# imazen/image-webp

Hardware: AMD Instinct MI355X
Metric: 1920x1080 lossy encodes/s (Q75, method 4) (higher is better)
Workload: dtype int32; 1 GPU; encode_frame_lossy 1920x1080 RGBA Q75 m4; device_batch=1024, distinct_frames=4, mbs_per_frame=8160, parallelism=frames sharded over 1 GPU(s), steps_pipelined=True, pipeline_lanes=2

## Files before the change

image-webp_amd/csrc/zw_dev.h:

```cpp
#pragma once
#include <hip/hip_runtime.h>
#include <stdint.h>
#include "zw_common.h"

#define ZW_TABLE(T, N, D, ...) __constant__ T d_##N D = {__VA_ARGS__};
#include "zw_tables.inc"
#undef ZW_TABLE

__constant__ uint8_t d_I4_IDX[10][16] = {
    {255, 255, 255, 255, 255, 255, 255, 255, 255, 255, 255, 255, 255, 255, 255, 255},
    {254, 254, 254, 254, 254, 254, 254, 254, 254, 254, 254, 254, 254, 254, 254, 254},
    {17, 18, 19, 20, 17, 18, 19, 20, 17, 18, 19, 20, 17, 18, 19, 20},
    {15, 15, 15, 15, 14, 14, 14, 14, 13, 13, 13, 13, 37, 37, 37, 37},
    {18, 19, 20, 21, 19, 20, 21, 22, 20, 21, 22, 23, 21, 22, 23, 36},
    {16, 17, 18, 19, 15, 16, 17, 18, 14, 15, 16, 17, 13, 14, 15, 16},
    {28, 29, 30, 31, 16, 17, 18, 19, 15, 28, 29, 30, 14, 16, 17, 18},
    {29, 30, 31, 32, 18, 19, 20, 21, 30, 31, 32, 22, 19, 20, 21, 23},
    {27, 16, 17, 18, 26, 15, 27, 16, 25, 14, 26, 15, 24, 13, 25, 14},
    {26, 14, 25, 13, 25, 13, 24, 37, 24, 37, 0, 0, 0, 0, 0, 0},
};

#define DI __device__ __forceinline__

DI int kZZ(int n) { return (int)((0xfeb7adc963258410ull >> (4 * n)) & 15); }
DI int kBand(int n)
{
    return n >= 16 ? 0 : (int)((0x7666666665463210ull >> (4 * n)) & 15);
}
DI int kWTrellis(int j)
{
    const unsigned long long lo = 0x0a11181b0b131b1eull, hi = 0x06080a0b080c1113ull;
    return (int)(((j < 8 ? lo : hi) >> (8 * (j & 7))) & 255);
}
DI int kWY(int j)
{
    const unsigned long long lo = 0x07111c2009142026ull, hi = 0x02040709040a1114ull;
    return (int)(((j < 8 ? lo : hi) >> (8 * (j & 7))) & 255);
}

DI int band_of(int n)
{
    return n >= 16 ? 0 : (int)((0x7666666665463210ull >> (4 * n)) & 15);
}
DI int zz_of(int n) { return (int)((0xfeb7adc963258410ull >> (4 * n)) & 15); }
DI int izz_of(int k) { return (int)((0xfea9db83c7426510ull >> (4 * k)) & 15); }

DI int clamp255(int v) { return v < 0 ? 0 : (v > 255 ? 255 : v); }
DI int iabs(int v) { return v < 0 ? -v : v; }

__device__ __forceinline__ int pk_y(uint32_t p)
{
    return (16839 * (int)(p & 255u) + 33059 * (int)((p >> 8) & 255u) + 6420 * (int)((p >> 16) & 255u) + (1 << 15) +
            (16 << 16)) >> 16;
}
__device__ __forceinline__ int pk_u(uint32_t p)
{
    return -9719 * (int)(p & 255u) - 19081 * (int)((p >> 8) & 255u) + 28800 * (int)((p >> 16) & 255u);
}
__device__ __forceinline__ int pk_v(uint32_t p)
{
    return 28800 * (int)(p & 255u) - 24116 * (int)((p >> 8) & 255u) - 4684 * (int)((p >> 16) & 255u);
}
__device__ __forceinline__ uint32_t udot2(uint32_t a, uint32_t b, uint32_t c)
{
    uint32_t d;
    asm("v_dot2_u32_u16 %0, %1, %2, %3" : "=v"(d) : "v"(a), "v"(b), "v"(c));
    return d;
}
__device__ __forceinline__ int sdot2(uint32_t a, uint32_t b, int c)
{
    int d;
    asm("v_dot2_i32_i16 %0, %1, %2, %3" : "=v"(d) : "v"(a), "v"(b), "v"(c));
    return d;
}
__device__ __forceinline__ uint32_t pk_y2(uint32_t p)
{
    const uint32_t rg = __builtin_amdgcn_perm(0u, p, 0x0c010c00u);
    return udot2(rg, 0x812341c7u , ((p >> 16) & 255u) * 6420u + (1u << 15) + (16u << 16)) >> 16;
}
__device__ __forceinline__ uint32_t pk_y4(uint32_t p0, uint32_t p1, uint32_t p2, uint32_t p3)
{
    auto y = [](uint32_t p) {
        const uint32_t hi = __builtin_amdgcn_udot4(p, 0x00198141u, 0u, false);
        const uint32_t lo = __builtin_amdgcn_udot4(p, 0x001423c7u, (1u << 15) + (16u << 16), false);
        return (hi << 8) + lo;
    };
    const uint32_t lo = __builtin_amdgcn_perm(y(p1), y(p0), 0x0c0c0602u);
    const uint32_t hi = __builtin_amdgcn_perm(y(p3), y(p2), 0x06020c0cu);
    return lo | hi;
}
__device__ __forceinline__ void pk_uv4(uint32_t a, uint32_t b, uint32_t c, uint32_t d, uint32_t& u, uint32_t& v)
{
    const uint32_t sel = 0x0c020c00u;
    const uint32_t rb = __builtin_amdgcn_perm(0u, a, sel) + __builtin_amdgcn_perm(0u, b, sel) +
                        __builtin_amdgcn_perm(0u, c, sel) + __builtin_amdgcn_perm(0u, d, sel);
    const int g = (int)(((a >> 8) & 255u) + ((b >> 8) & 255u) + ((c >> 8) & 255u) + ((d >> 8) & 255u));
    const int su = sdot2(rb, 0x7080da09u , g * -19081 + (512 << 16));
    const int sv = sdot2(rb, 0xedb47080u , g * -24116 + (512 << 16));
    u = (uint32_t)((su + (1 << 17)) >> 18);
    v = (uint32_t)((sv + (1 << 17)) >> 18);
}

DI void wsync()
// ... 117 lines not shown
        b[r * 4] = w16(a + d) >> 3;
        b[r * 4 + 1] = w16(bb + c) >> 3;
        b[r * 4 + 2] = w16(bb - c) >> 3;
        b[r * 4 + 3] = w16(a - d) >> 3;
    }
}

DI void wht16(int* b)
{
#pragma unroll
    for (int i = 0; i < 4; i++) {
        int a = b[i * 4] + b[i * 4 + 3], bb = b[i * 4 + 1] + b[i * 4 + 2];
        int c = b[i * 4 + 1] - b[i * 4 + 2], d = b[i * 4] - b[i * 4 + 3];
        b[i * 4] = a + bb;
        b[i * 4 + 1] = c + d;
        b[i * 4 + 2] = a - bb;
        b[i * 4 + 3] = d - c;
    }
#pragma unroll
    for (int i = 0; i < 4; i++) {
        int a1 = b[i] + b[i + 12], b1 = b[i + 4] + b[i + 8];
        int c1 = b[i + 4] - b[i + 8], d1 = b[i] - b[i + 12];
        int a2 = a1 + b1, b2 = c1 + d1, c2 = a1 - b1, d2 = d1 - c1;
        b[i] = (a2 + (a2 > 0 ? 1 : 0)) / 2;
        b[i + 4] = (b2 + (b2 > 0 ? 1 : 0)) / 2;
        b[i + 8] = (c2 + (c2 > 0 ? 1 : 0)) / 2;
        b[i + 12] = (d2 + (d2 > 0 ? 1 : 0)) / 2;
    }
}

DI void iwht16(int* b)
{
#pragma unroll
    for (int i = 0; i < 4; i++) {
        int a1 = b[i] + b[12 + i], b1 = b[4 + i] + b[8 + i];
        int c1 = b[4 + i] - b[8 + i], d1 = b[i] - b[12 + i];
        b[i] = a1 + b1;
        b[4 + i] = c1 + d1;
        b[8 + i] = a1 - b1;
        b[12 + i] = d1 - c1;
    }
#pragma unroll
    for (int r = 0; r < 4; r++) {
        int a1 = b[4 * r] + b[4 * r + 3], b1 = b[4 * r + 1] + b[4 * r + 2];
        int c1 = b[4 * r + 1] - b[4 * r + 2], d1 = b[4 * r] - b[4 * r + 3];
        b[4 * r] = (a1 + b1 + 3) >> 3;
        b[4 * r + 1] = (c1 + d1 + 3) >> 3;
        b[4 * r + 2] = (a1 - b1 + 3) >> 3;
        b[4 * r + 3] = (d1 - c1 + 3) >> 3;
    }
}

DI int ttransform(const int* in)
{
    int tmp[16];
#pragma unroll
    for (int i = 0; i < 4; i++) {
        const int* r = in + i * 4;
        int a0 = r[0] + r[2], a1 = r[1] + r[3], a2 = r[1] - r[3], a3 = r[0] - r[2];
        tmp[i * 4] = a0 + a1;
        tmp[i * 4 + 1] = a3 + a2;
        tmp[i * 4 + 2] = a3 - a2;
        tmp[i * 4 + 3] = a0 - a1;
    }
    int sum = 0;
#pragma unroll
    for (int i = 0; i < 4; i++) {
        int a0 = tmp[i] + tmp[8 + i], a1 = tmp[4 + i] + tmp[12 + i];
        int a2 = tmp[4 + i] - tmp[12 + i], a3 = tmp[i] - tmp[8 + i];
        sum += kWY(i) * iabs(a0 + a1) + kWY(4 + i) * iabs(a3 + a2) +
               kWY(8 + i) * iabs(a3 - a2) + kWY(12 + i) * iabs(a0 - a1);
    }
    return sum;
}

struct LdsTables {
    uint16_t lc[4][8][3][68];
    uint16_t eob[4][8][3];
    uint16_t init[4][8][3];
    uint8_t probs[4][8][3][11];
    uint16_t lfc[2048];
    uint16_t ent[256];
    uint16_t fci4[10][10][10];
    uint8_t i4idx[10][16];
    uint8_t i4qa[10][16];
    uint8_t zz[16];
    uint8_t bands[17];
    uint8_t izz[16];
    uint8_t pad[15];
    uint16_t beob[4][8][3];
    uint16_t binit[4][8][3];
};

DI void load_static_tables(LdsTables* T, int tid, int nt, const uint8_t* probs )
{
    for (int i = tid; i < 96; i += nt) {
        const int p0 = probs[i * 11];
        (&T->beob[0][0][0])[i] = d_VP8_ENTROPY_COST[p0];
        (&T->binit[0][0][0])[i] = d_VP8_ENTROPY_COST[255 - p0];
    }
    for (int i = tid; i < 2048; i += nt) T->lfc[i] = d_VP8_LEVEL_FIXED_COSTS[i];
    for (int i = tid; i < 256; i += nt) T->ent[i] = d_VP8_ENTROPY_COST[i];
    for (int i = tid; i < 1000; i += nt) (&T->fci4[0][0][0])[i] = (&d_VP8_FIXED_COSTS_I4[0][0][0])[i];
    for (int i = tid; i < 160; i += nt) {
        const int idx = (&d_I4_IDX[0][0])[i], p = i & 15;
        (&T->i4idx[0][0])[i] = (uint8_t)idx;
        (&T->i4qa[0][0])[i] = (uint8_t)(4 * (idx == 254 ? 3 - (p >> 2) : (idx == 255 ? 38 : idx)));
    }
    for (int i = tid; i < 16; i += nt) T->zz[i] = d_ZIGZAG[i];
    for (int i = tid; i < 17; i += nt) T->bands[i] = d_VP8_ENC_BANDS[i];
    for (int i = tid; i < 16; i += nt) T->izz[d_ZIGZAG[i]] = (uint8_t)i;
}

DI uint32_t bitcost(const LdsTables* T, int bit, int p) { return bit ? T->ent[255 - p] : T->ent[p]; }

template <int FIRST>
DI uint32_t rcost(const int* c, int ctx0, int ctype, const LdsTables* T)
{
    int last = -1;
#pragma unroll
    for (int n = 0; n < 16; n++)
        if (c[n] != 0) last = n;
    const int p0 = T->probs[ctype][kBand(FIRST)][ctx0][0];
    if (last < 0) return bitcost(T, 0, p0);
    uint32_t cost = ctx0 == 0 ? bitcost(T, 1, p0) : 0;
    int ctx = ctx0;
#pragma unroll
    for (int n = FIRST; n < 16; n++) {
        if (n <= last) {
            int v = iabs(c[n]);
            cost += T->lfc[v < 2047 ? v : 2047] + T->lc[ctype][kBand(n)][ctx][v < 67 ? v : 67];
            ctx = v < 2 ? v : 2;
        }
    }
    if (last < 15) cost += bitcost(T, 0, T->probs[ctype][band_of(last + 1)][ctx][0]);
    return cost;
}

#define DPP(v, ctrl) __builtin_amdgcn_mov_dpp((v), (ctrl), 0xf, 0xf, false)
DI int qb0(int v) { return DPP(v, 0x00); }
DI int qb1(int v) { return DPP(v, 0x55); }
DI int qb2(int v) { return DPP(v, 0xAA); }
DI int qb3(int v) { return DPP(v, 0xFF); }
DI int ror4(int v) { return DPP(v, 0x124); }
DI int ror8(int v) { return DPP(v, 0x128); }
DI int ror12(int v) { return DPP(v, 0x12C); }
DI int shr1(int v) { return __builtin_amdgcn_update_dpp(0, (v), 0x111, 0xf, 0xf, false); }
DI int red16(int v)
{
    v += DPP(v, 0xB1);
    v += DPP(v, 0x4E);
    v += DPP(v, 0x141);
    v += DPP(v, 0x140);
    return v;
}
DI int gget(int v, int k) { return __shfl(v, k, 16); }

DI int csel(bool c, int a, int b) { return b + ((a - b) & -(int)c); }

DI int sel4(int i, int a, int b, int c, int d)
{
    const int m0 = -(int)(i == 0), m1 = -(int)(i == 1), m2 = -(int)(i == 2), m3 = -(int)(i == 3);
    return (a & m0) | (b & m1) | (c & m2) | (d & m3);
}

DI void gcol(int t, int i, int& t0, int& t1, int& t2, int& t3)
{
    const int m1 = ror4(t), p2 = ror8(t), p1 = ror12(t);
    t0 = sel4(i, t, m1, p2, p1);
    t1 = sel4(i, p1, t, m1, p2);
    t2 = sel4(i, p2, p1, t, m1);
    t3 = sel4(i, m1, p2, p1, t);
}

DI int qrev(int v) { return DPP(v, 0x1B); }
DI int qnext(int v) { return DPP(v, 0x39); }
DI int qprev(int v) { return DPP(v, 0x93); }
DI int qxor2(int v) { return DPP(v, 0x4E); }
DI int rrev(int v) { return DPP(DPP(v, 0x140), 0x1B); }

DI int fdct_g(int v, int k)
{
    const int i = k >> 2, j = k & 3;
    {
        const int r = qrev(v);
        const int s = v + r, d = v - r;
        const int X = qnext(s), Y = qprev(d);
        const int ev = csel(j == 0, s + X, X - s) * 8;
        const int od = (m24(Y, 8 * 5352) + m24(d, csel(j == 1, 8 * 2217, -8 * 2217)) + csel(j == 1, 14500, 7500)) >> 12;
        v = csel((j & 1) == 0, ev, od);
// ... 532 lines not shown
```

image-webp_amd/csrc/zw_enc_i4pair.h:

```cpp
#pragma once
#include <stdint.h>

#ifndef ZW_HD
#ifdef __HIPCC__
#define ZW_HD __host__ __device__
#else
#define ZW_HD
#endif
#endif

#ifndef ZW_I4P_INV
#define ZW_I4P_INV 1
#endif
#ifndef ZW_I4P_LANES
#define ZW_I4P_LANES 1
#endif

#define ZW_I4P_KMAX 4

ZW_HD inline int i4p_inv_dest(int lane, int rank)
{
    return (lane & ~15) + (rank < ZW_I4P_KMAX ? 4 * rank : 1);
}
ZW_HD inline int i4p_mode_src(int lane) { return lane & ~3; }
ZW_HD inline bool i4p_eligible(int lane, int K) { return ((lane >> 2) & 3) < K; }
ZW_HD inline int i4p_mode(int lane, int K, int received) { return i4p_eligible(lane, K) ? received : 0; }

struct I4PWin {
    uint32_t pk;
    uint32_t sm;
};
ZW_HD inline I4PWin i4p_win(uint32_t rate, uint32_t mcost, bool nz, uint32_t sse, int mode)
{
    I4PWin w;
    w.pk = (rate & 0xffffu) | (mcost << 16) | ((uint32_t)nz << 31);
    w.sm = sse | ((uint32_t)mode << 24);
    return w;
}

struct I4PState {
    uint64_t running;
    uint32_t total_mc;
    uint32_t nzt;
    uint32_t lm;
};

ZW_HD inline void i4p_state_init(I4PState& s, uint32_t l_mode)
{
    s.running = 211ull * l_mode;
    s.total_mc = 0;
    s.nzt = 0;
    s.lm = 0;
}

ZW_HD inline void i4p_state_update(I4PState& s, int bx, int by, I4PWin w, uint32_t l_mode)
{
    const uint32_t mode = w.sm >> 24, sse = w.sm & 0xffffffu;
    s.nzt |= (w.pk >> 31) << (by * 4 + bx);
    s.nzt = (s.nzt & ~(0xf0000u << (4 * bx))) | (mode << (16 + 4 * bx));
    s.lm = (s.lm & ~(0xfu << (4 * by))) | (mode << (4 * by));
    s.total_mc += (w.pk >> 16) & 0x7fffu;
    s.running += (uint64_t)sse * 256ull + (uint64_t)(w.pk & 0xffffu) * l_mode;
}

ZW_HD inline int i4p_tctx(const I4PState& s, int bx, int by)
{
    return by == 0 ? 0 : (int)((s.nzt >> (16 + 4 * bx)) & 15u);
}
ZW_HD inline int i4p_lctx(const I4PState& s, int bx, int by)
{
    return bx == 0 ? 0 : (int)((s.lm >> (4 * by)) & 15u);
}
ZW_HD inline int i4p_nzctx(const I4PState& s, int bx, int by)
{
    const int i = by * 4 + bx;
    return (by == 0 ? 0 : (int)((s.nzt >> ((i - 4) & 15)) & 1u)) + (bx == 0 ? 0 : (int)((s.nzt >> ((i - 1) & 15)) & 1u));
}

ZW_HD inline bool i4p_exit(const I4PState& s, uint64_t i16_score)
{
    return s.running >= i16_score || s.total_mc > 256u * 16u * 16u / 4u;
}
```

image-webp_amd/csrc/zw_enc_kernels.hip:

```cpp
#include "zw_dev.h"

#include <type_traits>

#include "zw_enc_rows.h"
#include "zw_enc_pairfinal.h"
#include "zw_enc_i4pair.h"

#define ZW_PH_N 28

#ifdef ZW_NW
#define ZW_NW1 ZW_NW
#define ZW_NW2 ZW_NW
#endif
#ifndef ZW_NW1
#define ZW_NW1 12
#endif
#ifndef ZW_NW2
#define ZW_NW2 12
#endif
#define NW_MAX (ZW_NW1 > ZW_NW2 ? ZW_NW1 : ZW_NW2)
#ifndef ZW_DYN_PRIO
#define ZW_DYN_PRIO 1
#endif
#ifndef ZW_DYN_PRIO1
// ... 228 lines not shown
#ifdef ZW_PHASE_PROF
__device__ unsigned long long zw_phase_cycles_dev[2][ZW_PH_N];
__device__ unsigned long long zw_wave_cycles_dev[2][16][ZW_PH_N];
#define PH_START() long long ph_t_ = clock64()
#define PH_RESET() (ph_t_ = clock64())
#define PH_MARK(k) PH_MARK_L(k, lane, PASS)
#define PH_MARK_L(k, ln, ps)                                                        \
    do {                                                                            \
        const long long n_ = clock64();                                             \
        if ((ln) == 0) C.W->ph[k] += (unsigned long long)(n_ - ph_t_);               \
        ph_t_ = n_;                                                                 \
    } while (0)
extern "C" int zw_wave_cycles(unsigned long long* out, int reset)
{
    if (hipMemcpyFromSymbol(out, HIP_SYMBOL(zw_wave_cycles_dev), sizeof(zw_wave_cycles_dev)) != hipSuccess) return -1;
    if (reset) {
        static unsigned long long z[2][16][ZW_PH_N];
        if (hipMemcpyToSymbol(HIP_SYMBOL(zw_wave_cycles_dev), z, sizeof z) != hipSuccess) return -1;
    }
    return 0;
}
extern "C" int zw_phase_cycles(unsigned long long* out, int reset)
{
    if (hipMemcpyFromSymbol(out, HIP_SYMBOL(zw_phase_cycles_dev), sizeof(zw_phase_cycles_dev)) != hipSuccess) return -1;
    if (reset) {
        static unsigned long long z[2][ZW_PH_N];
        if (hipMemcpyToSymbol(HIP_SYMBOL(zw_phase_cycles_dev), z, sizeof z) != hipSuccess) return -1;
    }
    return 0;
}
#define PH_COUNT(k) \
    do {                \
        if (C.lane == 0) C.W->ph[k] += 1; \
    } while (0)
#else
#define PH_COUNT(k) (void)0
#define PH_START() (void)0
#define PH_RESET() (void)0
#define PH_MARK(k) (void)0
#define PH_MARK_L(k, ln, ps) (void)0
#endif

template <int NB>
__device__ __forceinline__ void i4_values_n(const Ctx& C, const int* x0, const int* y0)
{
    WaveLds* W = C.W;
    const uint8_t* ws = C.M->ws;
    const int l = C.lane;
    const int t = (int)(l >= 13) + (int)(l >= 24) + (int)(l >= 36) + (int)(l >= 37);
    const int k = min(l - 13 * (int)(l >= 13) - 11 * (int)(l >= 24), 12);
    const int t3 = (int)(t == 3), t4 = (int)(t >= 4), t12 = (int)(t == 1 || t == 2);
    const int ka = k + t3 * (11 - k) + t4 * (1 - k);
    const int kb = k + t12 + t3 * (12 - k) - t4 * k;
    const int kc = min(k + 2 * (int)(t == 1), 12);
    const int wb = 2 * (int)(t == 1) + (int)(t == 2) + 3 * (t3 + t4);
    const int wc = (int)(t == 1);
    const int sh = (int)(t != 0) + (int)(t != 0 && t != 2);
    const int oa = csel(ka < 4, -ka * ZW_BPS, ka - 4 - 4 * ZW_BPS);
    const int ob = csel(kb < 4, -kb * ZW_BPS, kb - 4 - 4 * ZW_BPS);
    const int oc = csel(kc < 4, -kc * ZW_BPS, kc - 4 - 4 * ZW_BPS);
    const bool dcl = l < 4 || (l >= 5 && l < 9);
    int v[NB], ea[NB];
#pragma unroll
    for (int h = 0; h < NB; h++) {
        const int rowL = (y0[h] + 3) * ZW_BPS + x0[h] - 1;
        ea[h] = ws[rowL + oa];
        const int eb = ws[rowL + ob], ec = ws[rowL + oc];
        v[h] = (ea[h] + wb * eb + wc * ec + ((1 << sh) >> 1)) >> sh;
    }
#pragma unroll
    for (int h = 0; h < NB; h++) {
        const int dsum = red16(dcl ? ea[h] : 0);
        if (l < 38) W->V[h][l] = v[h];
        if (l == 0) W->V[h][38] = (dsum + 4) >> 3;
    }
    wsync();
}
__device__ __forceinline__ void i4_values(const Ctx& C, int x0, int y0) { i4_values_n<1>(C, &x0, &y0); }

__device__ __forceinline__ int bperm(int v, int src_lane) { return __builtin_amdgcn_ds_bpermute(src_lane << 2, v); }

__device__ __forceinline__ int i4_src_index(const LdsTables* T, int mode, int p)
{
    const int idx = T->i4idx[mode][p];
    const bool tm = idx == 254;
    return csel(tm, 256 + 3 - (p >> 2), csel(idx == 255, 38, idx));
}
__device__ __forceinline__ int i4_pred_at(const int* V, int sidx, int vbc)
{
    const int va = V[sidx & 255];
    return csel(sidx >= 256, clamp255(va + vbc), va);
}

__device__ __forceinline__ unsigned long long rdscore(uint32_t sse, uint32_t rate, uint32_t lambda)
{
    return (unsigned long long)sse * 256ull + (unsigned long long)(uint16_t)rate * lambda;
}

struct I4State {
    unsigned long long running;
    uint32_t total_mc;
    unsigned long long mpack;
    uint32_t tnz, lnz;
    uint32_t nzm;
};

DI uint32_t min16u(uint32_t v)
{
    v = min(v, (uint32_t)DPP((int)v, 0x128));
    v = min(v, (uint32_t)DPP((int)v, 0x124));
    v = min(v, (uint32_t)DPP((int)v, 0x122));
    v = min(v, (uint32_t)DPP((int)v, 0x121));
    return v;
}

__device__ __forceinline__ int hx_partner(int v)
{
    const auto r = __builtin_amdgcn_permlane32_swap(v, v, false, false);
    return (__lane_id() < 32) ? (int)r[1] : (int)r[0];
}
__device__ __forceinline__ int hx_sum(int v)
{
    const auto r = __builtin_amdgcn_permlane32_swap(v, v, false, false);
    return (int)r[0] + (int)r[1];
}
DI int lo16(uint32_t v) { return (int)(int16_t)(v & 0xffffu); }
DI int hi16(uint32_t v) { return (int)(int16_t)(v >> 16); }

DI void uv_rows_pk(const uint8_t* w, const uint8_t* sblk, int bx, int by, int h, int m, int dc, uint32_t s01[2],
                   uint32_t s32[2], uint32_t p01[2], uint32_t p32[2])
{
    const int cm = -(int)(m & 1), rm = -(int)(m >= 2);
    const int P = w[0];
    const int ro = csel(m == 0, dc, csel(m == 3, -P, 0));
    const uint8_t* tp = w + 1 + bx * 4;
    const uint32_t c01 = pack_lo(tp[0] & cm, tp[1] & cm), c32 = pack_lo(tp[3] & cm, tp[2] & cm);
#pragma unroll
    for (int r = 0; r < 2; r++) {
        const int y = 2 * h + r;
        const int rv = (w[(by * 4 + y + 1) * ZW_BPS] & rm) + ro;
        const uint32_t rvv = pack_lo(rv, rv);
        p01[r] = clamp_pk(add_pk(c01, rvv));
        p32[r] = clamp_pk(add_pk(c32, rvv));
        const uint32_t sw = *(const uint32_t*)(sblk + y * 8);
        s01[r] = __builtin_amdgcn_perm(0u, sw, 0x0c010c00u);
        s32[r] = __builtin_amdgcn_perm(0u, sw, 0x0c020c03u);
    }
}

DI void fdct_pair(const uint32_t s01[2], const uint32_t s32[2], const uint32_t p01[2], const uint32_t p32[2], int h,
                  int cf[2][4])
{
    const zs2 k8p = {8, 8}, k8m = {8, -8}, k1a = {10704, 4434}, k1b = {4434, -10704};
    const uint32_t kA0 = h ? as_zu(k8m) : as_zu(k8p), kA1 = h ? as_zu(k8p) : as_zu(k8m);
    const uint32_t kD0 = h ? as_zu(k1b) : as_zu(k1a), kD1 = h ? as_zu(k1a) : as_zu(k1b);
    const int rD0 = h ? 1875 : 3625, rD1 = h ? 3625 : 1875;
    int own0[2], own1[2], oth0[2], oth1[2];
#pragma unroll
    for (int r = 0; r < 2; r++) {
        const uint32_t R01 = sub_pk(s01[r], p01[r]), R32 = sub_pk(s32[r], p32[r]);
        const uint32_t A = add_pk(R01, R32), D = sub_pk(R01, R32);
        own0[r] = dot2v(A, kA0, 0);
        oth0[r] = dot2v(A, kA1, 0);
        own1[r] = dot2v(D, kD0, rD0) >> 10;
        oth1[r] = dot2v(D, kD1, rD1) >> 10;
    }
    const uint32_t g0 = (uint32_t)hx_partner((int)pack_lo(oth0[0], oth0[1]));
    const uint32_t g1 = (uint32_t)hx_partner((int)pack_lo(oth1[0], oth1[1]));
    const zs2 k1p = {1, 1}, k1m = {1, -1}, k2a = {5352, 2217}, k2b = {2217, -5352};
// ... 523 lines not shown
    const uint32_t score = (uint32_t)sse * 256u + (rate & 0xffffu) * S.l_i4;
    const bool elig = m < 10 && rank < K;
    const uint32_t sk = elig ? score : 0xffffffffu;
    const uint32_t smin = min16u(sk);
    const uint32_t rk = sk == smin ? (uint32_t)rank : 0xffffffffu;
    const uint32_t rmin = min16u(rk);
    const unsigned long long win = __ballot(rk == rmin && sk == smin);
    PH_MARK_L(12, l, 0);
    int bmode[NB];
#pragma unroll
    for (int h = 0; h < NB; h++) {
        bmode[h] = __builtin_ctz((uint32_t)(win >> (16 * h)) & 0xffffu);
        const int wl = 16 * h + bmode[h];
        const uint32_t bsse = (uint32_t)__builtin_amdgcn_readlane(sse, wl);
        const uint32_t brate = (uint32_t)__builtin_amdgcn_readlane((int)rate, wl);
        const int bnz = __builtin_amdgcn_readlane((int)(last >= 0), wl);
        const int i = sby[h] * 4 + sbx[h];
        st.tnz = (st.tnz & ~(1u << sbx[h])) | ((uint32_t)bnz << sbx[h]);
        st.lnz = (st.lnz & ~(1u << sby[h])) | ((uint32_t)bnz << sby[h]);
        st.nzm |= (uint32_t)bnz << i;
        st.total_mc += (uint32_t)__builtin_amdgcn_readlane(mcost, wl);
        st.running += rdscore(bsse, brate, S.l_mode);
        st.mpack |= (unsigned long long)bmode[h] << (4 * i);
        if (l == h) C.M->modes[i] = (uint8_t)bmode[h];
    }
    const int bms = csel(slot, bmode[sl], bmode[0]);
    if (m == bms && (NB == 2 || slot == 0)) {
        const int xo = csel(slot, x0[sl], x0[0]), yo = csel(slot, y0[sl], y0[0]);
#pragma unroll
        for (int r = 0; r < 2; r++) {
            const uint32_t wd = __builtin_amdgcn_perm(r32[r], r01[r], 0x04060200u);
            uint8_t* p = C.M->ws + (yo + 2 * hf + r) * ZW_BPS + xo;
#pragma unroll
            for (int j = 0; j < 4; j++) p[j] = (uint8_t)(wd >> (8 * j));
        }
        if (keep) {
            int16_t* lv = C.M->lev[by * 4 + bx];
#pragma unroll
            for (int c = 0; c < 2; c++)
#pragma unroll
                for (int r = 0; r < 4; r++) {
                    const int a = av[c][r];
                    lv[izz_of(4 * r + 2 * hf + c)] = (int16_t)(((sgn >> (4 * c + r)) & 1u) ? -a : a);
                }
        }
    }
    wsync();
    PH_MARK_L(13, l, 0);
}

template <int PASS>
__device__ bool pick_i4(const Ctx& C, unsigned long long i16_score, bool keep, uint32_t& nzm)
{
    const ZwSegment& S = *C.S;
    const int K = C.method <= 3 ? 3 : (C.method == 4 ? 4 : 10);
    I4State st;
    st.running = 211ull * S.l_mode;
    st.total_mc = 0;
    st.mpack = 0;
    st.tnz = st.lnz = st.nzm = 0;
    I4Lane LC;
    i4_lane_init(C, LC);
    PH_COUNT(20);
    for (int s = 0; s < 10; s++) {
        PH_COUNT(19);
        const int sbyA = s < 4 ? 0 : (s - 2) >> 1;
        const int sbxA = s - 2 * sbyA;
        if (s >= 2 && s <= 7) {
            const int bx[2] = {sbxA, sbxA - 2}, by[2] = {sbyA, sbyA + 1};
            i4_step<PASS, 2>(C, bx, by, K, LC, st, keep);
        } else {
            i4_step<PASS, 1>(C, &sbxA, &sbyA, K, LC, st, keep);
        }
        if (st.running >= i16_score) return false;
        if (st.total_mc > 256u * 16u * 16u / 4u) return false;
    }
    nzm = st.nzm;
    return true;
}

struct I4PLane {
    uint32_t ix[4];
    uint32_t psel;
    int tm;
    uint32_t iq0, bs0, iq1, bs1;
    int q0, qa;
    uint32_t l_i4;
};

DI uint32_t i4p_psel(int hm, int slot)
{
    const uint32_t b = (uint32_t)(2 * hm + slot);
    return 0x0c000c00u | ((4u + b) << 16) | b;
}

DI void i4p_lane_init(const Ctx& C, const Ctx& CB, I4PLane& L)
{
    const int l = C.lane, m = l & 15, mv = m < 10 ? m : 0;
    {
        const ZwSegment* Sh = (l >> 5) ? CB.S : C.S;
        const int q = l & 3;
        L.iq0 = q ? Sh->y1.iq[1] : Sh->y1.iq[0];
        L.bs0 = q ? Sh->y1.bias[1] : Sh->y1.bias[0];
        L.iq1 = Sh->y1.iq[1];
        L.bs1 = Sh->y1.bias[1];
        L.q0 = q ? (int)Sh->y1.q[1] : (int)Sh->y1.q[0];
        L.qa = (int)Sh->y1.q[1];
        L.l_i4 = Sh->l_i4;
    }
#pragma unroll
    for (int r = 0; r < 4; r++) {
        uint32_t w = 0;
#pragma unroll
        for (int j = 0; j < 4; j++) w |= (uint32_t)(4 * (i4_src_index(C.T, mv, 4 * r + j) & 255)) << (8 * j);
        L.ix[r] = w;
    }
    L.psel = i4p_psel(l >> 5, (l >> 4) & 1);
    L.tm = mv == 1;
}

template <int NB>
DI uint32_t i4p_values(const Ctx& CA, const Ctx& CB, const int* x0, const int* y0)
{
    const int l = CA.lane;
    const int t = (int)(l >= 13) + (int)(l >= 24) + (int)(l >= 36) + (int)(l >= 37);
    const int k = min(l - 13 * (int)(l >= 13) - 11 * (int)(l >= 24), 12);
    const int t3 = (int)(t == 3), t4 = (int)(t >= 4), t12 = (int)(t == 1 || t == 2);
    const int ka = k + t3 * (11 - k) + t4 * (1 - k);
    const int kb = k + t12 + t3 * (12 - k) - t4 * k;
    const int kc = min(k + 2 * (int)(t == 1), 12);
    const int wb = 2 * (int)(t == 1) + (int)(t == 2) + 3 * (t3 + t4);
    const int wc = (int)(t == 1);
    const int sh = (int)(t != 0) + (int)(t != 0 && t != 2);
    const int oa = csel(ka < 4, -ka * ZW_BPS, ka - 4 - 4 * ZW_BPS);
    const int ob = csel(kb < 4, -kb * ZW_BPS, kb - 4 - 4 * ZW_BPS);
    const int oc = csel(kc < 4, -kc * ZW_BPS, kc - 4 - 4 * ZW_BPS);
    const bool dcl = l < 4 || (l >= 5 && l < 9);
    uint32_t v[2], ea[2];
#pragma unroll
    for (int mb = 0; mb < 2; mb++) {
        const uint8_t* ws = (mb ? CB : CA).M->ws;
        v[mb] = ea[mb] = 0;
#pragma unroll
        for (int h = 0; h < 2; h++) {
            const int hh = NB == 2 ? h : 0;
            const int rowL = (y0[hh] + 3) * ZW_BPS + x0[hh] - 1;
            const int a = ws[rowL + oa], eb = ws[rowL + ob], ec = ws[rowL + oc];
            v[mb] |= (uint32_t)((a + wb * eb + wc * ec + ((1 << sh) >> 1)) >> sh) << (16 * h);
            ea[mb] |= (uint32_t)a << (16 * h);
        }
    }
    const uint32_t da = (uint32_t)__builtin_amdgcn_readfirstlane(red16((int)(dcl ? ea[0] : 0u)));
    const uint32_t db = (uint32_t)__builtin_amdgcn_readfirstlane(red16((int)(dcl ? ea[1] : 0u)));
    const uint32_t dcv = (((da & 0xffffu) + 4) >> 3) | ((((da >> 16) + 4) >> 3) << 8) |
                         ((((db & 0xffffu) + 4) >> 3) << 16) | ((((db >> 16) + 4) >> 3) << 24);
    return l == 38 ? dcv : __builtin_amdgcn_perm(v[1], v[0], 0x06040200u);
}

#if ZW_I4P_LANES
typedef I4PState I4PSearch;
#else
struct I4PSearch {
    I4State mb[2];
};
#endif

template <int PASS, int NB>
DI void i4p_step(const Ctx& CA, const Ctx& CB, const int* sbx, const int* sby, int K, const I4PLane& LC,
                 I4PSearch& st, const bool act[2], bool keep)
{
    [[maybe_unused]] const Ctx& C = CA;
    const int l = CA.lane, m = l & 15, hm = l >> 5;
    const int slot = NB == 2 ? (l >> 4) & 1 : 0;
    const int sl = NB == 2 ? 1 : 0;
    int x0[NB], y0[NB];
#pragma unroll
    for (int h = 0; h < NB; h++) {
        x0[h] = sbx[h] * 4 + 1;
        y0[h] = sby[h] * 4 + 1;
    }
    const int bx = csel(slot, sbx[sl], sbx[0]), by = csel(slot, sby[sl], sby[0]);
#if ZW_I4P_LANES
    const int tctx = i4p_tctx(st, bx, by), lctx = i4p_lctx(st, bx, by), ctx0 = i4p_nzctx(st, bx, by);
#else
    int tc[2][NB], lc[2][NB], nc[2][NB];
#pragma unroll
    for (int h = 0; h < NB; h++) {
        const int i = sby[h] * 4 + sbx[h];
#pragma unroll
        for (int mb = 0; mb < 2; mb++) {
            tc[mb][h] = sby[h] == 0 ? 0 : (int)((st.mb[mb].mpack >> (4 * (i - 4))) & 15);
            lc[mb][h] = sbx[h] == 0 ? 0 : (int)((st.mb[mb].mpack >> (4 * (i - 1))) & 15);
            nc[mb][h] = (sby[h] == 0 ? 0 : (int)((st.mb[mb].tnz >> sbx[h]) & 1)) +
                        (sbx[h] == 0 ? 0 : (int)((st.mb[mb].lnz >> sby[h]) & 1));
        }
    }
    auto pick = [&](const int (&v)[2][NB]) {
        const int a = csel(slot, v[0][sl], v[0][0]), b = csel(slot, v[1][sl], v[1][0]);
        return csel(hm, b, a);
    };
    const int tctx = pick(tc), lctx = pick(lc), ctx0 = pick(nc);
#endif
    const uint8_t* sYh = hm ? CB.sY : CA.sY;
    const LdsTables* Th = hm ? CB.T : CA.T;
    const int k = (l >> 2) & 3, q = l & 3;
    int hn[2];
    uint32_t swq;
    const uint16_t* fcrow;
    auto read_ctx = [&]() {
        hn[0] = (int)Th->binit[3][0][ctx0] & -(int)(ctx0 == 0);
        hn[1] = (int)Th->beob[3][0][ctx0];
        swq = *(const uint32_t*)(sYh + (by * 4 + q) * 16 + bx * 4);
        fcrow = Th->fci4[tctx][lctx];
    };
    PH_START();
    const uint32_t vp = i4p_values<NB>(CA, CB, x0, y0);
    uint32_t ap01, ap32;
    {
        const uint32_t P = (uint32_t)__builtin_amdgcn_readlane((int)vp, 4);
        uint32_t a[4];
#pragma unroll
        for (int j = 0; j < 4; j++) a[j] = (uint32_t)__builtin_amdgcn_readlane((int)vp, 5 + j);
        const int sh = 8 * (2 * hm + slot);
        const int p_ = (int)((P >> sh) & 255u);
        const int d0 = (int)((a[0] >> sh) & 255u) - p_, d1 = (int)((a[1] >> sh) & 255u) - p_;
        const int d2 = (int)((a[2] >> sh) & 255u) - p_, d3 = (int)((a[3] >> sh) & 255u) - p_;
        ap01 = pack_lo(d0, d1);
        ap32 = pack_lo(d3, d2);
    }
    PH_MARK_L(10, l, 0);
#if ZW_I4P_INV
    read_ctx();
#endif
    int pse = 0;
#pragma unroll
    for (int r = 0; r < 4; r++) {
        const uint32_t ix = LC.ix[r];
        const uint32_t v0 = (uint32_t)__builtin_amdgcn_ds_bpermute((int)(ix & 255u), (int)vp);
        const uint32_t v1 = (uint32_t)__builtin_amdgcn_ds_bpermute((int)((ix >> 8) & 255u), (int)vp);
        const uint32_t v2 = (uint32_t)__builtin_amdgcn_ds_bpermute((int)((ix >> 16) & 255u), (int)vp);
        const uint32_t v3 = (uint32_t)__builtin_amdgcn_ds_bpermute((int)(ix >> 24), (int)vp);
        const uint32_t q01 = __builtin_amdgcn_perm(v1, v0, LC.psel), q32 = __builtin_amdgcn_perm(v2, v3, LC.psel);
        const uint32_t p01 = LC.tm ? clamp_pk(add_pk(q01, ap01)) : q01;
        const uint32_t p32 = LC.tm ? clamp_pk(add_pk(q32, ap32)) : q32;
        const uint32_t sw = *(const uint32_t*)(sYh + (by * 4 + r) * 16 + bx * 4);
        const uint32_t d01 = sub_pk(__builtin_amdgcn_perm(0u, sw, 0x0c010c00u), p01);
        const uint32_t d32 = sub_pk(__builtin_amdgcn_perm(0u, sw, 0x0c020c03u), p32);
        pse = dot2v(d01, d01, pse);
        pse = dot2v(d32, d32, pse);
    }
    const int key = m < 10 ? (pse << 4) | m : 0x7fffffff;
    const int rank = rank16(key);
    PH_MARK_L(11, l, 0);
#if ZW_I4P_INV
    const int mv = i4p_mode(l, K, qb0(__builtin_amdgcn_ds_permute(4 * i4p_inv_dest(l, rank), m)));
#else
    unsigned long long modes = 0;
    for (int kk = 0; kk < K; kk++) {
        const unsigned long long b = __ballot(m < 10 && rank == kk);
#pragma unroll
        for (int g = 0; g < 4; g++)
            modes |= (unsigned long long)__builtin_ctz((uint32_t)(b >> (16 * g)) | 0x10000u) << (16 * g + 4 * kk);
    }
    const int mq = (int)((modes >> (16 * (2 * hm + slot) + 4 * k)) & 15ull);
    const int mv = k < K ? mq : 0;
    read_ctx();
#endif
    const int mcost = fcrow[mv];
    const uint32_t iq0 = LC.iq0, bs0 = LC.bs0, iq1 = LC.iq1, bs1 = LC.bs1;
    const int q0 = LC.q0, qa = LC.qa;
    uint32_t p01, p32;
    {
        const uint32_t iw = *(const uint32_t*)&Th->i4qa[mv][4 * q];
        uint32_t v[4];
#pragma unroll
        for (int j = 0; j < 4; j++)
            v[j] = (uint32_t)__builtin_amdgcn_ds_bpermute((int)((iw >> (8 * j)) & 255u), (int)vp);
        const uint32_t q01 = __builtin_amdgcn_perm(v[1], v[0], LC.psel), q32 = __builtin_amdgcn_perm(v[2], v[3], LC.psel);
        const bool tm = mv == 1;
        p01 = tm ? clamp_pk(add_pk(q01, ap01)) : q01;
        p32 = tm ? clamp_pk(add_pk(q32, ap32)) : q32;
    }
    const uint32_t s01 = __builtin_amdgcn_perm(0u, swq, 0x0c010c00u);
    const uint32_t s32 = __builtin_amdgcn_perm(0u, swq, 0x0c020c03u);
    PH_MARK_L(22, l, 0);
    const uint32_t R01 = sub_pk(s01, p01), R32 = sub_pk(s32, p32);
    int cf[4];
    uvq_fdct(add_pk(R01, R32), sub_pk(R01, R32), q, cf);
    int av[4], dq[4], lv[4];
#pragma unroll
    for (int r = 0; r < 4; r++) {
        const bool dcs = r == 0;
        const int v = cf[r];
        const int a = (int)((__umul24((uint32_t)iabs(v), dcs ? iq0 : iq1) + (dcs ? bs0 : bs1)) >> 17);
        av[r] = a;
        lv[r] = v < 0 ? -a : a;
        dq[r] = m24(lv[r], dcs ? q0 : qa);
    }
    int last;
    const int cost = rcost_quad<PASS == 2>(av, q, ctx0, 3, Th, last, hn);
    PH_MARK_L(23, l, 0);
    uint32_t r01, r32;
    uvq_idct_recon(dq, p01, p32, q, r01, r32);
    int sse = 0;
    {
        const uint32_t d01 = sub_pk(s01, r01), d32 = sub_pk(s32, r32);
        sse = dot2v(d01, d01, sse);
        sse = dot2v(d32, d32, sse);
    }
    sse = quad_sum(sse);
    const uint32_t rate = (uint32_t)(mcost + cost);
    const uint32_t score = (uint32_t)sse * 256u + (rate & 0xffffu) * LC.l_i4;
    const uint32_t key2 = k < K ? (score << 2) | (uint32_t)k : 0xffffffffu;
    const uint32_t kmin = min16u(key2);
    const bool actl = hm ? act[1] : act[0];
#if ZW_I4P_LANES
    const bool winl = key2 == kmin && k < K;
    PH_MARK_L(12, l, 0);
    {
        const I4PWin own = i4p_win(rate, (uint32_t)mcost, last >= 0, (uint32_t)sse, mv);
        uint32_t w0 = winl ? own.pk : 0u, w1 = winl ? own.sm : 0u;
        w0 |= (uint32_t)ror8((int)w0);
        w1 |= (uint32_t)ror8((int)w1);
        w0 |= (uint32_t)ror4((int)w0);
        w1 |= (uint32_t)ror4((int)w1);
        const uint32_t lml = hm ? CB.S->l_mode : CA.S->l_mode;
        if (NB == 2) {
            const auto p0 = __builtin_amdgcn_permlane16_swap(w0, w0, false, false);
            const auto p1 = __builtin_amdgcn_permlane16_swap(w1, w1, false, false);
#pragma unroll
            for (int h = 0; h < 2; h++) {
                I4PWin w;
                w.pk = p0[h];
                w.sm = p1[h];
                i4p_state_update(st, sbx[h], sby[h], w, lml);
            }
        } else {
            I4PWin w;
            w.pk = w0;
            w.sm = w1;
            i4p_state_update(st, sbx[0], sby[0], w, lml);
        }
        if (actl && m == 0 && ((l >> 4) & 1) < NB) (hm ? CB.M : CA.M)->modes[by * 4 + bx] = (uint8_t)(w1 >> 24);
    }
#else
    const unsigned long long win = __ballot(key2 == kmin);
    const uint32_t pk = (rate & 0xffffu) | ((uint32_t)mcost << 16) | ((uint32_t)(last >= 0) << 31);
    PH_MARK_L(12, l, 0);
#pragma unroll
    for (int mb = 0; mb < 2; mb++) {
        const ZwSegment& S = *(mb ? CB : CA).S;
        MbLds* M = (mb ? CB : CA).M;
#pragma unroll
        for (int h = 0; h < NB; h++) {
            const int gg = 2 * mb + h;
            const int bk = __builtin_ctz((uint32_t)(win >> (16 * gg)) & 0xffffu) >> 2;
            const int wl = 16 * gg + 4 * bk;
#if ZW_I4P_INV
            const int bmode = __builtin_amdgcn_readlane(mv, wl);
#else
            const int bmode = (int)((modes >> (16 * gg + 4 * bk)) & 15ull);
#endif
            const uint32_t bsse = (uint32_t)__builtin_amdgcn_readlane(sse, wl);
            const uint32_t bpk = (uint32_t)__builtin_amdgcn_readlane((int)pk, wl);
// ... 1854 lines not shown
```

Before: 4981 encodes/s.

## Precompute TM predictor values per lane and rank I4 modes with udot4 SSE

Extends the per-lane I4 predictor value vector so that TrueMotion predictions are computed and clamped once in dedicated lanes (39-54), replacing per-candidate add/clamp work. Replaces the packed 16-bit difference dot products for mode ranking with byte udot4 accumulation of p·p and s·p, ranking on p²-2sp, which is SSE minus a mode-independent term. A new i4qp table holds the permute indices. This trims ALU work in the hot I4 search at the cost of more value-lane setup and a changed ranking key that must preserve ordering.

```diff
diff --git a/image-webp_amd/csrc/zw_dev.h b/image-webp_amd/csrc/zw_dev.h
--- a/image-webp_amd/csrc/zw_dev.h
+++ b/image-webp_amd/csrc/zw_dev.h
@@ -2,23 +2,13 @@
 #include <hip/hip_runtime.h>
 #include <stdint.h>
 #include "zw_common.h"
+#include "zw_enc_i4pair.h"
 
 #define ZW_TABLE(T, N, D, ...) __constant__ T d_##N D = {__VA_ARGS__};
 #include "zw_tables.inc"
 #undef ZW_TABLE
 
-__constant__ uint8_t d_I4_IDX[10][16] = {
-    {255, 255, 255, 255, 255, 255, 255, 255, 255, 255, 255, 255, 255, 255, 255, 255},
-    {254, 254, 254, 254, 254, 254, 254, 254, 254, 254, 254, 254, 254, 254, 254, 254},
-    {17, 18, 19, 20, 17, 18, 19, 20, 17, 18, 19, 20, 17, 18, 19, 20},
-    {15, 15, 15, 15, 14, 14, 14, 14, 13, 13, 13, 13, 37, 37, 37, 37},
-    {18, 19, 20, 21, 19, 20, 21, 22, 20, 21, 22, 23, 21, 22, 23, 36},
-    {16, 17, 18, 19, 15, 16, 17, 18, 14, 15, 16, 17, 13, 14, 15, 16},
-    {28, 29, 30, 31, 16, 17, 18, 19, 15, 28, 29, 30, 14, 16, 17, 18},
-    {29, 30, 31, 32, 18, 19, 20, 21, 30, 31, 32, 22, 19, 20, 21, 23},
-    {27, 16, 17, 18, 26, 15, 27, 16, 25, 14, 26, 15, 24, 13, 25, 14},
-    {26, 14, 25, 13, 25, 13, 24, 37, 24, 37, 0, 0, 0, 0, 0, 0},
-};
+__constant__ uint8_t d_I4_IDX[10][16] = {ZW_I4_IDX_ROWS};
 
 #define DI __device__ __forceinline__
 
@@ -302,8 +292,8 @@
     uint16_t lfc[2048];
     uint16_t ent[256];
     uint16_t fci4[10][10][10];
-    uint8_t i4idx[10][16];
     uint8_t i4qa[10][16];
+    uint8_t i4qp[10][16];
     uint8_t zz[16];
     uint8_t bands[17];
     uint8_t izz[16];
@@ -324,8 +314,8 @@
     for (int i = tid; i < 1000; i += nt) (&T->fci4[0][0][0])[i] = (&d_VP8_FIXED_COSTS_I4[0][0][0])[i];
     for (int i = tid; i < 160; i += nt) {
         const int idx = (&d_I4_IDX[0][0])[i], p = i & 15;
-        (&T->i4idx[0][0])[i] = (uint8_t)idx;
         (&T->i4qa[0][0])[i] = (uint8_t)(4 * (idx == 254 ? 3 - (p >> 2) : (idx == 255 ? 38 : idx)));
+        (&T->i4qp[0][0])[i] = (uint8_t)(4 * i4p_vindex(idx, p));
     }
     for (int i = tid; i < 16; i += nt) T->zz[i] = d_ZIGZAG[i];
     for (int i = tid; i < 17; i += nt) T->bands[i] = d_VP8_ENC_BANDS[i];
diff --git a/image-webp_amd/csrc/zw_enc_i4pair.h b/image-webp_amd/csrc/zw_enc_i4pair.h
--- a/image-webp_amd/csrc/zw_enc_i4pair.h
+++ b/image-webp_amd/csrc/zw_enc_i4pair.h
@@ -16,7 +16,94 @@
 #define ZW_I4P_LANES 1
 #endif
 
+#ifndef ZW_I4P_TMV
+#define ZW_I4P_TMV 1
+#endif
+#ifndef ZW_I4P_DOT4
+#define ZW_I4P_DOT4 1
+#endif
+
 #define ZW_I4P_KMAX 4
+
+#define ZW_I4P_NV (ZW_I4P_TMV ? 55 : 39)
+#define ZW_I4P_V_DC 38
+#define ZW_I4P_V_TM 39
+
+#define ZW_I4_IDX_ROWS \
+    {255, 255, 255, 255, 255, 255, 255, 255, 255, 255, 255, 255, 255, 255, 255, 255}, \
+    {254, 254, 254, 254, 254, 254, 254, 254, 254, 254, 254, 254, 254, 254, 254, 254}, \
+    {17, 18, 19, 20, 17, 18, 19, 20, 17, 18, 19, 20, 17, 18, 19, 20}, \
+    {15, 15, 15, 15, 14, 14, 14, 14, 13, 13, 13, 13, 37, 37, 37, 37}, \
+    {18, 19, 20, 21, 19, 20, 21, 22, 20, 21, 22, 23, 21, 22, 23, 36}, \
+    {16, 17, 18, 19, 15, 16, 17, 18, 14, 15, 16, 17, 13, 14, 15, 16}, \
+    {28, 29, 30, 31, 16, 17, 18, 19, 15, 28, 29, 30, 14, 16, 17, 18}, \
+    {29, 30, 31, 32, 18, 19, 20, 21, 30, 31, 32, 22, 19, 20, 21, 23}, \
+    {27, 16, 17, 18, 26, 15, 27, 16, 25, 14, 26, 15, 24, 13, 25, 14}, \
+    {26, 14, 25, 13, 25, 13, 24, 37, 24, 37, 0, 0, 0, 0, 0, 0},
+
+struct I4PValue {
+    int ka, kb, kc;
+    int wb, wc, sh;
+};
+ZW_HD inline I4PValue i4p_value_map(int l)
+{
+    const int t = (int)(l >= 13) + (int)(l >= 24) + (int)(l >= 36) + (int)(l >= 37);
+    const int k0 = l - 13 * (int)(l >= 13) - 11 * (int)(l >= 24), k = k0 < 12 ? k0 : 12;
+    const int t3 = (int)(t == 3), t4 = (int)(t >= 4), t12 = (int)(t == 1 || t == 2);
+    const int kc0 = k + 2 * (int)(t == 1);
+    I4PValue v;
+    v.ka = k + t3 * (11 - k) + t4 * (1 - k);
+    v.kb = k + t12 + t3 * (12 - k) - t4 * k;
+    v.kc = kc0 < 12 ? kc0 : 12;
+    v.wb = 2 * (int)(t == 1) + (int)(t == 2) + 3 * (t3 + t4);
+    v.wc = (int)(t == 1);
+    v.sh = (int)(t != 0) + (int)(t != 0 && t != 2);
+#if ZW_I4P_TMV
+    const bool t5 = l >= ZW_I4P_V_TM;
+    const int i = l - ZW_I4P_V_TM, r = (i >> 2) & 3, j = i & 3;
+    v.ka = t5 ? 3 - r : v.ka;
+    v.kb = t5 ? 5 + j : v.kb;
+    v.kc = t5 ? 4 : v.kc;
+    v.wb = t5 ? 1 : v.wb;
+    v.wc = t5 ? -1 : v.wc;
+    v.sh = t5 ? 0 : v.sh;
+#endif
+    return v;
+}
+ZW_HD inline int i4p_value(const I4PValue& v, int ea, int eb, int ec)
+{
+    const int x = (ea + v.wb * eb + v.wc * ec + ((1 << v.sh) >> 1)) >> v.sh;
+#if ZW_I4P_TMV
+    return x < 0 ? 0 : (x > 255 ? 255 : x);
+#else
+    return x;
+#endif
+}
+ZW_HD inline bool i4p_value_dc_term(int l) { return l < 4 || (l >= 5 && l < 9); }
+
+ZW_HD inline int i4p_vindex(int idx, int p)
+{
+    return idx == 254 ? (ZW_I4P_TMV ? ZW_I4P_V_TM + p : 3 - (p >> 2)) : (idx == 255 ? ZW_I4P_V_DC : idx);
+}
+
+ZW_HD inline uint32_t i4p_psel(int hm, int slot)
+{
+    const uint32_t b = (uint32_t)(2 * hm + slot);
+    return 0x0c000c00u | ((4u + b) << 16) | b;
+}
+ZW_HD inline uint32_t i4p_bsel(int hm, int slot)
+{
+    const uint32_t b = (uint32_t)(2 * hm + slot);
+    return 0x0c0c0000u | ((4u + b) << 8) | b;
+}
+ZW_HD inline uint32_t i4p_pack_row(uint32_t b01, uint32_t b23) { return (b23 << 16) | b01; }
+#define ZW_I4P_PAIRS_TO_ROW 0x04060200u
+
+#define ZW_I4P_KEY_BIAS (1u << 22)
+ZW_HD inline uint32_t i4p_rank_key(uint32_t pp, uint32_t sp, int m)
+{
+    return ((ZW_I4P_KEY_BIAS + pp - 2u * sp) << 4) | (uint32_t)m;
+}
 
 ZW_HD inline int i4p_inv_dest(int lane, int rank)
 {
diff --git a/image-webp_amd/csrc/zw_enc_kernels.hip b/image-webp_amd/csrc/zw_enc_kernels.hip
--- a/image-webp_amd/csrc/zw_enc_kernels.hip
+++ b/image-webp_amd/csrc/zw_enc_kernels.hip
@@ -334,9 +334,7 @@
 
 __device__ __forceinline__ int i4_src_index(const LdsTables* T, int mode, int p)
 {
-    const int idx = T->i4idx[mode][p];
-    const bool tm = idx == 254;
-    return csel(tm, 256 + 3 - (p >> 2), csel(idx == 255, 38, idx));
+    return (T->i4qa[mode][p] >> 2) + csel(mode == 1, 256, 0);
 }
 __device__ __forceinline__ int i4_pred_at(const int* V, int sidx, int vbc)
 {
@@ -1026,17 +1024,16 @@
 struct I4PLane {
     uint32_t ix[4];
     uint32_t psel;
+#if ZW_I4P_DOT4 && ZW_I4P_TMV
+    uint32_t bsel;
+#endif
+#if !ZW_I4P_TMV
     int tm;
+#endif
     uint32_t iq0, bs0, iq1, bs1;
     int q0, qa;
     uint32_t l_i4;
 };
-
-DI uint32_t i4p_psel(int hm, int slot)
-{
-    const uint32_t b = (uint32_t)(2 * hm + slot);
-    return 0x0c000c00u | ((4u + b) << 16) | b;
-}
 
 DI void i4p_lane_init(const Ctx& C, const Ctx& CB, I4PLane& L)
 {
@@ -1053,33 +1050,25 @@
         L.l_i4 = Sh->l_i4;
     }
 #pragma unroll
-    for (int r = 0; r < 4; r++) {
-        uint32_t w = 0;
-#pragma unroll
-        for (int j = 0; j < 4; j++) w |= (uint32_t)(4 * (i4_src_index(C.T, mv, 4 * r + j) & 255)) << (8 * j);
-        L.ix[r] = w;
-    }
+    for (int r = 0; r < 4; r++) L.ix[r] = *(const uint32_t*)&C.T->i4qp[mv][4 * r];
     L.psel = i4p_psel(l >> 5, (l >> 4) & 1);
+#if ZW_I4P_DOT4 && ZW_I4P_TMV
+    L.bsel = i4p_bsel(l >> 5, (l >> 4) & 1);
+#endif
+#if !ZW_I4P_TMV
     L.tm = mv == 1;
+#endif
 }
 
 template <int NB>
 DI uint32_t i4p_values(const Ctx& CA, const Ctx& CB, const int* x0, const int* y0)
 {
     const int l = CA.lane;
-    const int t = (int)(l >= 13) + (int)(l >= 24) + (int)(l >= 36) + (int)(l >= 37);
-    const int k = min(l - 13 * (int)(l >= 13) - 11 * (int)(l >= 24), 12);
-    const int t3 = (int)(t == 3), t4 = (int)(t >= 4), t12 = (int)(t == 1 || t == 2);
-    const int ka = k + t3 * (11 - k) + t4 * (1 - k);
-    const int kb = k + t12 + t3 * (12 - k) - t4 * k;
-    const int kc = min(k + 2 * (int)(t == 1), 12);
-    const int wb = 2 * (int)(t == 1) + (int)(t == 2) + 3 * (t3 + t4);
-    const int wc = (int)(t == 1);
-    const int sh = (int)(t != 0) + (int)(t != 0 && t != 2);
-    const int oa = csel(ka < 4, -ka * ZW_BPS, ka - 4 - 4 * ZW_BPS);
-    const int ob = csel(kb < 4, -kb * ZW_BPS, kb - 4 - 4 * ZW_BPS);
-    const int oc = csel(kc < 4, -kc * ZW_BPS, kc - 4 - 4 * ZW_BPS);
-    const bool dcl = l < 4 || (l >= 5 && l < 9);
+    const I4PValue vm = i4p_value_map(l);
+    const int oa = csel(vm.ka < 4, -vm.ka * ZW_BPS, vm.ka - 4 - 4 * ZW_BPS);
+    const int ob = csel(vm.kb < 4, -vm.kb * ZW_BPS, vm.kb - 4 - 4 * ZW_BPS);
+    const int oc = csel(vm.kc < 4, -vm.kc * ZW_BPS, vm.kc - 4 - 4 * ZW_BPS);
+    const bool dcl = i4p_value_dc_term(l);
     uint32_t v[2], ea[2];
 #pragma unroll
     for (int mb = 0; mb < 2; mb++) {
@@ -1090,7 +1079,7 @@
             const int hh = NB == 2 ? h : 0;
             const int rowL = (y0[hh] + 3) * ZW_BPS + x0[hh] - 1;
             const int a = ws[rowL + oa], eb = ws[rowL + ob], ec = ws[rowL + oc];
-            v[mb] |= (uint32_t)((a + wb * eb + wc * ec + ((1 << sh) >> 1)) >> sh) << (16 * h);
+            v[mb] |= (uint32_t)i4p_value(vm, a, eb, ec) << (16 * h);
             ea[mb] |= (uint32_t)a << (16 * h);
         }
     }
@@ -1098,7 +1087,7 @@
     const uint32_t db = (uint32_t)__builtin_amdgcn_readfirstlane(red16((int)(dcl ? ea[1] : 0u)));
     const uint32_t dcv = (((da & 0xffffu) + 4) >> 3) | ((((da >> 16) + 4) >> 3) << 8) |
                          ((((db & 0xffffu) + 4) >> 3) << 16) | ((((db >> 16) + 4) >> 3) << 24);
-    return l == 38 ? dcv : __builtin_amdgcn_perm(v[1], v[0], 0x06040200u);
+    return l == ZW_I4P_V_DC ? dcv : __builtin_amdgcn_perm(v[1], v[0], 0x06040200u);
 }
 
 #if ZW_I4P_LANES
@@ -1159,6 +1148,7 @@
     };
     PH_START();
     const uint32_t vp = i4p_values<NB>(CA, CB, x0, y0);
+#if !ZW_I4P_TMV
     uint32_t ap01, ap32;
     {
         const uint32_t P = (uint32_t)__builtin_amdgcn_readlane((int)vp, 4);
@@ -1172,11 +1162,16 @@
         ap01 = pack_lo(d0, d1);
         ap32 = pack_lo(d3, d2);
     }
+#endif
     PH_MARK_L(10, l, 0);
 #if ZW_I4P_INV
     read_ctx();
 #endif
+#if ZW_I4P_DOT4
+    uint32_t pp = 0, sp = 0;
+#else
     int pse = 0;
+#endif
 #pragma unroll
     for (int r = 0; r < 4; r++) {
         const uint32_t ix = LC.ix[r];
@@ -1184,16 +1179,37 @@
         const uint32_t v1 = (uint32_t)__builtin_amdgcn_ds_bpermute((int)((ix >> 8) & 255u), (int)vp);
         const uint32_t v2 = (uint32_t)__builtin_amdgcn_ds_bpermute((int)((ix >> 16) & 255u), (int)vp);
         const uint32_t v3 = (uint32_t)__builtin_amdgcn_ds_bpermute((int)(ix >> 24), (int)vp);
+        const uint32_t sw = *(const uint32_t*)(sYh + (by * 4 + r) * 16 + bx * 4);
+#if ZW_I4P_DOT4 && ZW_I4P_TMV
+        const uint32_t b01 = __builtin_amdgcn_perm(v1, v0, LC.bsel), b23 = __builtin_amdgcn_perm(v3, v2, LC.bsel);
+        const uint32_t pw = i4p_pack_row(b01, b23);
+#else
         const uint32_t q01 = __builtin_amdgcn_perm(v1, v0, LC.psel), q32 = __builtin_amdgcn_perm(v2, v3, LC.psel);
+#if ZW_I4P_TMV
+        const uint32_t p01 = q01, p32 = q32;
+#else
         const uint32_t p01 = LC.tm ? clamp_pk(add_pk(q01, ap01)) : q01;
         const uint32_t p32 = LC.tm ? clamp_pk(add_pk(q32, ap32)) : q32;
-        const uint32_t sw = *(const uint32_t*)(sYh + (by * 4 + r) * 16 + bx * 4);
+#endif
+#if ZW_I4P_DOT4
+        const uint32_t pw = __builtin_amdgcn_perm(p32, p01, ZW_I4P_PAIRS_TO_ROW);
+#endif
+#endif
+#if ZW_I4P_DOT4
+        pp = __builtin_amdgcn_udot4(pw, pw, pp, false);
+        sp = __builtin_amdgcn_udot4(sw, pw, sp, false);
+#else
         const uint32_t d01 = sub_pk(__builtin_amdgcn_perm(0u, sw, 0x0c010c00u), p01);
         const uint32_t d32 = sub_pk(__builtin_amdgcn_perm(0u, sw, 0x0c020c03u), p32);
         pse = dot2v(d01, d01, pse);
         pse = dot2v(d32, d32, pse);
-    }
+#endif
+    }
+#if ZW_I4P_DOT4
+    const int key = m < 10 ? (int)i4p_rank_key(pp, sp, m) : 0x7fffffff;
+#else
     const int key = m < 10 ? (pse << 4) | m : 0x7fffffff;
+#endif
     const int rank = rank16(key);
     PH_MARK_L(11, l, 0);
 #if ZW_I4P_INV
@@ -1215,15 +1231,20 @@
     const int q0 = LC.q0, qa = LC.qa;
     uint32_t p01, p32;
     {
-        const uint32_t iw = *(const uint32_t*)&Th->i4qa[mv][4 * q];
+        const uint32_t iw = *(const uint32_t*)&Th->i4qp[mv][4 * q];
         uint32_t v[4];
 #pragma unroll
         for (int j = 0; j < 4; j++)
             v[j] = (uint32_t)__builtin_amdgcn_ds_bpermute((int)((iw >> (8 * j)) & 255u), (int)vp);
         const uint32_t q01 = __builtin_amdgcn_perm(v[1], v[0], LC.psel), q32 = __builtin_amdgcn_perm(v[2], v[3], LC.psel);
+#if ZW_I4P_TMV
+        p01 = q01;
+        p32 = q32;
+#else
         const bool tm = mv == 1;
         p01 = tm ? clamp_pk(add_pk(q01, ap01)) : q01;
         p32 = tm ? clamp_pk(add_pk(q32, ap32)) : q32;
+#endif
     }
     const uint32_t s01 = __builtin_amdgcn_perm(0u, swq, 0x0c010c00u);
     const uint32_t s32 = __builtin_amdgcn_perm(0u, swq, 0x0c020c03u);
```

Measured after the change: 5139 encodes/s (median of 6 runs). 3.2% higher.
